# Kamino666/S2VT-video-caption

Hardware: AMD Instinct MI355X
Metric: training frames/sec (whole node) (higher is better)
Workload: dtype f32; 1 GPU; BASELINE configs[1]: S2VT train step, B=64 per GPU x 1 GPU, 80x4096 feats, hidden=embed=1000, vocab=12000, fp32, Adam; global_batch=64, frames=80, parallelism=dp1

## Files before the change

include/s2vt_hip.h:

```cpp
#ifndef S2VT_HIP_H
#define S2VT_HIP_H

#include <stddef.h>
#include <stdint.h>

#ifdef __cplusplus
extern "C" {
#endif

#define S2VT_ABI_VERSION 9

#define S2VT_ERR_ARG (-1)
#define S2VT_ERR_INDEX (-2)
#define S2VT_ERR_TIMEOUT (-3)

typedef struct s2vt_dims {
    int32_t B, L, F, H, E, V;
} s2vt_dims;

typedef struct s2vt_params {
    const float* vid_w_ih;
    const float* vid_w_hh;
    const float* vid_b_ih;
    const float* vid_b_hh;
// ... 189 lines not shown
                        size_t workspace_bytes, void* stream);

size_t s2vt_lstm_seq_bf16_workspace_bytes(int32_t T, int32_t B, int32_t H);
int s2vt_lstm_seq_fwd_bf16(int32_t T, int32_t B, int32_t H, float* gx_stash, int32_t n_gx, const float* bias,
                           const float* w_hh, float* h_all, float* c_all, void* workspace, size_t workspace_bytes,
                           int32_t persistent, int32_t block, void* stream);
int s2vt_lstm_seq_fwd_bf16_pair(int32_t T, int32_t B, int32_t H, float* gx_stash0, float* gx_stash1, int32_t n_gx,
                                const float* bias0, const float* bias1, const float* w_hh0, const float* w_hh1,
                                float* h_all0, float* h_all1, float* c_all0, float* c_all1, void* workspace,
                                size_t workspace_bytes, int32_t block, void* stream);
size_t s2vt_lstm_seq_bwd_bf16_workspace_bytes(int32_t T, int32_t B, int32_t H);
int s2vt_lstm_seq_bwd_bf16(int32_t T, int32_t B, int32_t H, const float* w_hh, const float* dh_out, int32_t dh_first,
                           const float* c_all, float* stash_dg, void* workspace, size_t workspace_bytes,
                           int32_t persistent, int32_t block, void* stream);
int s2vt_lstm_seq_bwd_bf16_pair(int32_t T, int32_t B, int32_t H, const float* w_hh0, const float* w_hh1, const float* dh_out0,
                                const float* dh_out1, int32_t dh_first, const float* c_all0, const float* c_all1,
                                float* stash_dg0, float* stash_dg1, void* workspace, size_t workspace_bytes, int32_t block,
                                void* stream);
int s2vt_set_recurrence_mode(int32_t mode);
int s2vt_recurrence_plan(int32_t B, int32_t H, int32_t* fwd, int32_t* bwd);
int s2vt_decode_plan(const s2vt_dims* d, int32_t encode_only, int32_t* padded_B, int32_t* persist_encode, int32_t* schedule);

size_t s2vt_lstm_seq_x3_workspace_bytes(int32_t T, int32_t B, int32_t H);
int s2vt_lstm_seq_fwd_x3_persist(int32_t T, int32_t B, int32_t H, float* gx_stash0, float* gx_stash1, int32_t n_gx,
                              const float* bias0, const float* bias1, const float* w_hh0, const float* w_hh1, float* h_all0,
                              float* h_all1, float* c_all0, float* c_all1, int32_t block, void* workspace,
                              size_t workspace_bytes, void* stream);
size_t s2vt_lstm_seq_bwd_x3_workspace_bytes(int32_t T, int32_t B, int32_t H, int32_t block);
int s2vt_lstm_seq_bwd_x3_persist(int32_t T, int32_t B, int32_t H, const float* w_hh0, const float* w_hh1, const float* dh_out0,
                                 const float* dh_out1, int32_t dh_first, const float* c_all0, const float* c_all1, float* stash_dg0,
                                 float* stash_dg1, int32_t block, void* workspace, size_t workspace_bytes, void* stream);
int s2vt_decode_step_argmax(int32_t B, int32_t H, int32_t V, const float* h, const float* w_out, const float* b_out,
                            unsigned long long* packed, void* stream);

size_t s2vt_decode_step_argmax_x3_workspace_bytes(int32_t B, int32_t H, int32_t V);
int s2vt_decode_step_argmax_x3(int32_t B, int32_t H, int32_t V, const float* h, const float* w_out, const float* b_out,
                               unsigned long long* packed, void* workspace, size_t workspace_bytes, void* stream);

int s2vt_decode_step_sample(int32_t B, int32_t H, int32_t V, const float* h, const float* w_out, const float* b_out, float temperature,
                            uint64_t seed, int32_t step, int32_t row0, unsigned long long* packed, void* stream);
size_t s2vt_decode_step_sample_x3_workspace_bytes(int32_t B, int32_t H, int32_t V);
int s2vt_decode_step_sample_x3(int32_t B, int32_t H, int32_t V, const float* h, const float* w_out, const float* b_out, float temperature,
                               uint64_t seed, int32_t step, int32_t row0, unsigned long long* packed, void* workspace,
                               size_t workspace_bytes, void* stream);
int s2vt_sample_decode(const s2vt_dims* d, const s2vt_params* p, const float* feats, int32_t sos_ix, float temperature, uint64_t seed,
                       int64_t* ids, void* workspace, size_t workspace_bytes, void* stream);
int s2vt_sample_decode_cached(const s2vt_dims* d, const s2vt_params* p, const float* feats, int32_t sos_ix, float temperature,
                              uint64_t seed, int64_t* ids, void* workspace, size_t workspace_bytes, void* cache, size_t cache_bytes,
                              int32_t cache_valid, void* stream);

int s2vt_scheduled_decode(const s2vt_dims* d, const s2vt_params* p, const float* feats, const int64_t* targets, int64_t targets_ld,
                          float ss_prob, int32_t draw_mode, float temperature, uint64_t seed, int64_t* used, int64_t* draws,
                          void* workspace, size_t workspace_bytes, void* stream);
int s2vt_scheduled_decode_cached(const s2vt_dims* d, const s2vt_params* p, const float* feats, const int64_t* targets, int64_t targets_ld,
                                 float ss_prob, int32_t draw_mode, float temperature, uint64_t seed, int64_t* used, int64_t* draws,
                                 void* workspace, size_t workspace_bytes, void* cache, size_t cache_bytes, int32_t cache_valid,
                                 void* stream);
int s2vt_ss_mix(const int64_t* draw_tokens, const int64_t* targets, int64_t targets_ld, int32_t B, float ss_prob, uint64_t seed,
                int32_t step, int32_t row0, int64_t* out, void* stream);
int s2vt_ss_unpack(const unsigned long long* packed, int32_t steps, int32_t B, const int64_t* targets, int64_t targets_ld, float ss_prob,
                   uint64_t seed, int64_t* used, int64_t* draws, void* stream);

int32_t s2vt_set_option(const char* name, int32_t value);
int32_t s2vt_option_count(void);
const char* s2vt_option_name(int32_t index);

int s2vt_set_gemm_mode(int32_t mode);

int s2vt_set_pipeline_block(int32_t steps);
int s2vt_set_decode_schedule(int32_t schedule);
int s2vt_decode_encode_cached(const s2vt_dims* d, const s2vt_params* p, const float* feats, void* workspace, size_t workspace_bytes,
                              void* cache, size_t cache_bytes, int32_t cache_valid, float* vid_h, float* vid_c, float* word_h,
                              float* word_c, float* gx_dec, int32_t depth, void* stream);
int s2vt_beam_step_gx(const s2vt_dims* d, const s2vt_params* p, int32_t R, const int32_t* row_b, const int32_t* row_state,
                      const int32_t* tok, const float* gx_vid, const float* word_h_in, const float* word_c_in, float* word_h_out,
                      float* word_c_out, int32_t* top_ix, float* top_lp, void* workspace, size_t workspace_bytes, void* cache,
                      size_t cache_bytes, void* stream);
int s2vt_pipeline_overlaps(void);

int s2vt_set_graph_mode(int32_t on);
int s2vt_graph_stats(int64_t* captures, int64_t* replays);

int s2vt_test_occupy_cus(int32_t workgroups, int32_t lds_bytes, int64_t microseconds, void* stream);
int s2vt_test_lane_delay(int32_t lanes, int64_t microseconds);

int s2vt_prof_enable(int32_t on);
int s2vt_prof_read(int32_t kind, double* total_ms, int64_t* launches);
int s2vt_prof_read_busy(int32_t kind, double* busy_ms);
int s2vt_prof_reset(void);

#ifdef __cplusplus
}
#endif
#endif
```

s2vt-video-caption_amd/capi.py:

```python
import ctypes
import os
from ctypes import POINTER, c_char_p, c_double, c_float, c_int32, c_int64, c_size_t, c_uint64, c_void_p

_HERE = os.path.dirname(os.path.abspath(__file__))
LIB_PATH = os.environ.get("S2VT_LIB") or os.path.join(_HERE, "libs2vt_hip.so")


class Dims(ctypes.Structure):
    _fields_ = [(n, c_int32) for n in ("B", "L", "F", "H", "E", "V")]


PARAM_FIELDS = ("vid_w_ih", "vid_w_hh", "vid_b_ih", "vid_b_hh", "word_w_ih", "word_w_hh", "word_b_ih", "word_b_hh",
                "feat_w", "feat_b", "out_w", "out_b", "emb_w")
PARAM_KEYS = ("vid_rnn.weight_ih_l0", "vid_rnn.weight_hh_l0", "vid_rnn.bias_ih_l0", "vid_rnn.bias_hh_l0",
              "word_rnn.weight_ih_l0", "word_rnn.weight_hh_l0", "word_rnn.bias_ih_l0", "word_rnn.bias_hh_l0",
              "feat_linear.weight", "feat_linear.bias", "out_linear.weight", "out_linear.bias", "embedding.weight")


class Params(ctypes.Structure):
    _fields_ = [(n, c_void_p) for n in PARAM_FIELDS]


class Grads(ctypes.Structure):
    _fields_ = [(n, c_void_p) for n in PARAM_FIELDS]
# ... 69 lines not shown
    "s2vt_beam_queue_step": (c_int32, [c_int32] * 6 + [c_void_p, c_size_t] + [c_void_p] * 6),
    "s2vt_beam_queue_result": (c_int32, [c_int32, c_int32, c_int32, c_void_p, c_size_t, c_void_p, c_int32, c_void_p, c_void_p]),
    "s2vt_feat_proj_fwd": (c_int32, [POINTER(Dims), c_void_p, c_void_p, c_void_p, c_void_p, c_void_p]),
    "s2vt_feat_proj_bwd": (c_int32, [POINTER(Dims), c_void_p, c_void_p, c_void_p, c_void_p, c_void_p, c_void_p,
                                     c_void_p, c_void_p]),
    "s2vt_colsum_ws_floats": (c_size_t, [c_int64, c_int32]),
    "s2vt_lstm_step_fwd": (c_int32, [c_int32, c_int32] + [c_void_p] * 9),
    "s2vt_lstm_step_fwd_token": (c_int32, [c_int32, c_int32, c_int32, c_int32] + [c_void_p] * 6 + [c_int64, c_void_p, c_void_p,
                                                                                            c_int32, c_void_p, c_void_p, c_void_p]),
    "s2vt_lstm_step_bwd": (c_int32, [c_int32, c_int32] + [c_void_p] * 7 + [c_int32, c_void_p, c_void_p]),
    "s2vt_lstm_seq_fwd": (c_int32, [c_int32, c_int32, c_int32, c_void_p, c_int32] + [c_void_p] * 6),
    "s2vt_lstm_seq_bwd": (c_int32, [c_int32, c_int32, c_int32, c_void_p, c_void_p, c_int32] + [c_void_p] * 5),
    "s2vt_gru_step_fwd": (c_int32, [c_int32, c_int32] + [c_void_p] * 8),
    "s2vt_gru_step_fwd_token": (c_int32, [c_int32, c_int32, c_int32, c_int32] + [c_void_p] * 6 + [c_int64, c_void_p, c_void_p,
                                                                                           c_int32, c_void_p, c_void_p]),
    "s2vt_gru_step_bwd": (c_int32, [c_int32, c_int32] + [c_void_p] * 10),
    "s2vt_lstm_chain_fwd": (c_int32, [c_int32, c_int32, c_int32, c_int32, POINTER(LstmLayer), c_void_p]),
    "s2vt_lstm_chain_bwd_workspace_bytes": (c_size_t, [c_int32, c_int32, c_int32]),
    "s2vt_lstm_chain_bwd": (c_int32, [c_int32, c_int32, c_int32, c_int32, POINTER(LstmLayer), c_void_p, c_size_t, c_void_p]),
    "s2vt_gru_seq_fwd": (c_int32, [c_int32, c_int32, c_int32, c_void_p, c_int32] + [c_void_p] * 6),
    "s2vt_gru_seq_bwd": (c_int32, [c_int32, c_int32, c_int32, c_void_p, c_void_p, c_int32] + [c_void_p] * 7),
    "s2vt_tokens_time_major": (c_int32, [c_int32, c_int32, c_int32, c_void_p, c_int64, c_void_p, c_void_p]),
    "s2vt_lstm_seq_bf16_workspace_bytes": (c_size_t, [c_int32, c_int32, c_int32]),
    "s2vt_lstm_seq_fwd_bf16": (c_int32, [c_int32, c_int32, c_int32, c_void_p, c_int32, c_void_p, c_void_p, c_void_p,
                                         c_void_p, c_void_p, c_size_t, c_int32, c_int32, c_void_p]),
    "s2vt_lstm_seq_fwd_bf16_pair": (c_int32, [c_int32, c_int32, c_int32, c_void_p, c_void_p, c_int32] + [c_void_p] * 9 +
                                    [c_size_t, c_int32, c_void_p]),
    "s2vt_lstm_seq_bwd_bf16_workspace_bytes": (c_size_t, [c_int32, c_int32, c_int32]),
    "s2vt_lstm_seq_bwd_bf16": (c_int32, [c_int32, c_int32, c_int32, c_void_p, c_void_p, c_int32, c_void_p, c_void_p, c_void_p,
                                         c_size_t, c_int32, c_int32, c_void_p]),
    "s2vt_lstm_seq_bwd_bf16_pair": (c_int32, [c_int32, c_int32, c_int32, c_void_p, c_void_p, c_void_p, c_void_p, c_int32,
                                              c_void_p, c_void_p, c_void_p, c_void_p, c_void_p, c_size_t, c_int32, c_void_p]),
    "s2vt_lstm_seq_x3_workspace_bytes": (c_size_t, [c_int32, c_int32, c_int32]),
    "s2vt_lstm_seq_fwd_x3_persist": (c_int32, [c_int32, c_int32, c_int32, c_void_p, c_void_p, c_int32] + [c_void_p] * 8 +
                                  [c_int32, c_void_p, c_size_t, c_void_p]),
    "s2vt_lstm_seq_bwd_x3_workspace_bytes": (c_size_t, [c_int32, c_int32, c_int32, c_int32]),
    "s2vt_lstm_seq_bwd_x3_persist": (c_int32, [c_int32, c_int32, c_int32, c_void_p, c_void_p, c_void_p, c_void_p, c_int32] +
                                     [c_void_p] * 4 + [c_int32, c_void_p, c_size_t, c_void_p]),
    "s2vt_set_recurrence_mode": (c_int32, [c_int32]),
    "s2vt_recurrence_plan": (c_int32, [c_int32, c_int32, POINTER(c_int32), POINTER(c_int32)]),
    "s2vt_decode_plan": (c_int32, [POINTER(Dims), c_int32, POINTER(c_int32), POINTER(c_int32), POINTER(c_int32)]),
    "s2vt_decode_step_argmax": (c_int32, [c_int32, c_int32, c_int32] + [c_void_p] * 5),
    "s2vt_decode_step_argmax_x3_workspace_bytes": (c_size_t, [c_int32, c_int32, c_int32]),
    "s2vt_decode_step_argmax_x3": (c_int32, [c_int32, c_int32, c_int32] + [c_void_p] * 5 + [c_size_t, c_void_p]),
    "s2vt_decode_step_sample": (c_int32, [c_int32, c_int32, c_int32, c_void_p, c_void_p, c_void_p, c_float, c_uint64, c_int32, c_int32,
                                          c_void_p, c_void_p]),
    "s2vt_decode_step_sample_x3_workspace_bytes": (c_size_t, [c_int32, c_int32, c_int32]),
    "s2vt_decode_step_sample_x3": (c_int32, [c_int32, c_int32, c_int32, c_void_p, c_void_p, c_void_p, c_float, c_uint64, c_int32,
                                             c_int32, c_void_p, c_void_p, c_size_t, c_void_p]),
    "s2vt_sample_decode": (c_int32, [POINTER(Dims), POINTER(Params), c_void_p, c_int32, c_float, c_uint64, c_void_p, c_void_p,
                                     c_size_t, c_void_p]),
    "s2vt_sample_decode_cached": (c_int32, [POINTER(Dims), POINTER(Params), c_void_p, c_int32, c_float, c_uint64, c_void_p, c_void_p,
                                            c_size_t, c_void_p, c_size_t, c_int32, c_void_p]),
    "s2vt_scheduled_decode": (c_int32, [POINTER(Dims), POINTER(Params), c_void_p, c_void_p, c_int64, c_float, c_int32, c_float, c_uint64,
                                        c_void_p, c_void_p, c_void_p, c_size_t, c_void_p]),
    "s2vt_scheduled_decode_cached": (c_int32, [POINTER(Dims), POINTER(Params), c_void_p, c_void_p, c_int64, c_float, c_int32, c_float,
                                               c_uint64, c_void_p, c_void_p, c_void_p, c_size_t, c_void_p, c_size_t, c_int32, c_void_p]),
    "s2vt_ss_mix": (c_int32, [c_void_p, c_void_p, c_int64, c_int32, c_float, c_uint64, c_int32, c_int32, c_void_p, c_void_p]),
    "s2vt_ss_unpack": (c_int32, [c_void_p, c_int32, c_int32, c_void_p, c_int64, c_float, c_uint64, c_void_p, c_void_p, c_void_p]),
    "s2vt_gru_step_fwd_token_ss": (c_int32, [c_int32, c_int32, c_int32, c_int32] + [c_void_p] * 6 + [c_int64, c_void_p, c_void_p, c_int64,
                                                                                              c_float, c_uint64, c_int32, c_int32, c_void_p,
                                                                                              c_void_p]),
    "s2vt_weighted_ce_forward": (c_int32, [c_int32, c_int32, c_int32, c_void_p, c_void_p, c_int64, c_void_p, c_int64, c_void_p,
                                           c_void_p, c_void_p, c_void_p]),
    "s2vt_weighted_ce_backward": (c_int32, [c_int32, c_int32, c_int32, c_void_p, c_void_p, c_int64, c_void_p, c_int64, c_void_p,
                                            c_void_p, c_void_p, c_void_p, c_void_p]),
    "s2vt_cider_rewards": (c_int32, [POINTER(CiderTable), c_void_p, c_void_p, c_int32, c_int32, c_int64, c_int32, c_int32, c_void_p,
                                     c_void_p]),
    "s2vt_sc_weights": (c_int32, [c_void_p, c_void_p, c_void_p, c_int32, c_int32, c_int32, c_int32, c_void_p, c_void_p, c_void_p]),
    "s2vt_mean_ce_backward_fused": (c_int32, [POINTER(Dims), c_void_p, c_void_p, c_int64, c_void_p, c_void_p, c_void_p, c_size_t,
                                              c_void_p]),
    "s2vt_set_option": (c_int32, [c_char_p, c_int32]),
    "s2vt_option_count": (c_int32, []),
    "s2vt_option_name": (c_char_p, [c_int32]),
    "s2vt_set_gemm_mode": (c_int32, [c_int32]),
    "s2vt_set_pipeline_block": (c_int32, [c_int32]),
    "s2vt_set_decode_schedule": (c_int32, [c_int32]),
    "s2vt_decode_encode_cached": (c_int32, [POINTER(Dims), POINTER(Params), c_void_p, c_void_p, c_size_t, c_void_p, c_size_t, c_int32,
                                            c_void_p, c_void_p, c_void_p, c_void_p, c_void_p, c_int32, c_void_p]),
    "s2vt_beam_step_gx": (c_int32, [POINTER(Dims), POINTER(Params), c_int32] + [c_void_p] * 10 + [c_void_p, c_size_t, c_void_p, c_size_t,
                                                                                                  c_void_p]),
    "s2vt_pipeline_overlaps": (c_int32, []),
    "s2vt_test_occupy_cus": (c_int32, [c_int32, c_int32, c_int64, c_void_p]),
    "s2vt_test_lane_delay": (c_int32, [c_int32, c_int64]),
    "s2vt_set_graph_mode": (c_int32, [c_int32]),
    "s2vt_graph_stats": (c_int32, [POINTER(c_int64), POINTER(c_int64)]),
    "s2vt_prof_enable": (c_int32, [c_int32]),
    "s2vt_prof_read": (c_int32, [c_int32, POINTER(c_double), POINTER(c_int64)]),
    "s2vt_prof_read_busy": (c_int32, [c_int32, POINTER(c_double)]),
    "s2vt_prof_reset": (c_int32, []),
}

_lib = None


class S2VTHipError(RuntimeError):
    pass


def load():
    global _lib
    if _lib is not None:
        return _lib
    if not os.path.exists(LIB_PATH):
        raise S2VTHipError(
            "libs2vt_hip.so is not built (%s). Run `python -c 'import __graft_entry__ as g; g.build()'` "
            "or `python s2vt-video-caption_amd/build.py`. There is no CPU fallback for the S2VT hot path." % LIB_PATH)
    import torch
    rt = os.path.join(os.path.dirname(torch.__file__), "lib", "libamdhip64.so")
    if os.path.exists(rt):
        ctypes.CDLL(rt, mode=ctypes.RTLD_GLOBAL)
    lib = ctypes.CDLL(LIB_PATH)
    for name, (res, args) in SIGNATURES.items():
        fn = getattr(lib, name)
        fn.restype = res
        fn.argtypes = args
    if lib.s2vt_abi_version() != ABI_VERSION:
        raise S2VTHipError("libs2vt_hip.so ABI %d != %d" % (lib.s2vt_abi_version(), ABI_VERSION))
    _lib = lib
    return lib


ERR_INDEX, ERR_TIMEOUT = -2, -3


def check(rc, what):
    if rc != 0:
        msg = load().s2vt_last_error()
        text = "%s failed (rc=%d): %s" % (what, rc, msg.decode(errors="replace") if msg else "?")
        if rc == ERR_INDEX:
            raise IndexError(text)
        raise S2VTHipError(text)


def check_async_error(wait=True):
    check(load().s2vt_check_async_error(1 if wait else 0), "s2vt_check_async_error")


def prof_read_busy(kind):
    ms = c_double(0.0)
    check(load().s2vt_prof_read_busy(kind, ctypes.byref(ms)), "s2vt_prof_read_busy")
    return ms.value


def prof_read(kind):
    ms, n = c_double(0.0), c_int64(0)
    check(load().s2vt_prof_read(kind, ctypes.byref(ms), ctypes.byref(n)), "s2vt_prof_read")
    return ms.value, n.value


def recurrence_plan(B, H):
    import ctypes
    f, b = c_int32(0), c_int32(0)
    lib = load()
    check(lib.s2vt_recurrence_plan(int(lib.s2vt_padded_batch(int(B))), int(H), ctypes.byref(f), ctypes.byref(b)), "s2vt_recurrence_plan")
    return f.value, b.value


def decode_plan(dims, encode_only=False):
    d = dims if isinstance(dims, Dims) else Dims(*[int(x) for x in dims])
    b, pe, sc = c_int32(0), c_int32(0), c_int32(0)
    check(load().s2vt_decode_plan(d, 1 if encode_only else 0, ctypes.byref(b), ctypes.byref(pe), ctypes.byref(sc)), "s2vt_decode_plan")
    return b.value, pe.value, sc.value
```

s2vt-video-caption_amd/csrc/api_runtime.hip:

```cpp
#include "api_internal.h"

namespace s2vt {

static thread_local char g_err[512] = "";
const char* last_error_text() { return g_err; }
#ifdef S2VT_EXPERIMENT_STAMPS
unsigned long long* g_xstamps = nullptr;
int g_xstamp_block = 0;
#endif

void set_error(const char* fmt, ...) {
    va_list ap;
    va_start(ap, fmt);
    vsnprintf(g_err, sizeof(g_err), fmt, ap);
    va_end(ap);
}

int check_hip(hipError_t e, const char* what) {
    if (e == hipSuccess) return 0;
    set_error("%s: %s", what, hipGetErrorString(e));
    return (int)e;
}

struct ErrRecord { int* host; hipEvent_t ev; bool pending; };
// ... 183 lines not shown
        (void)hipEventSynchronize(e2);
        (void)hipEventElapsedTime(&single, e0, e2);
    }
    (void)hipEventDestroy(e0); (void)hipEventDestroy(e1); (void)hipEventDestroy(e2);
    return both < 1.6f * single;
}
static int g_side_overlaps = -1;
int side_stream_overlaps() { return g_side_overlaps; }
int side_stream(hipStream_t caller, hipStream_t* out) {
    if (!g_side) {
        hipStream_t cand = nullptr;
        g_side_overlaps = 0;
        for (int attempt = 0; attempt < 8 && !g_side_overlaps; ++attempt) {
            S2VT_HIP(hipStreamCreateWithFlags(&cand, hipStreamNonBlocking));
            if (streams_overlap(caller, cand)) g_side_overlaps = 1;
        }
        g_side = cand;
    }
    *out = g_side;
    return 0;
}
int get_event(size_t i, hipEvent_t* out) {
    while (g_events.size() <= i) {
        hipEvent_t e;
        S2VT_HIP(hipEventCreateWithFlags(&e, hipEventDisableTiming));
        g_events.push_back(e);
    }
    *out = g_events[i];
    return 0;
}
int handoff(hipStream_t from, hipStream_t to, size_t ev_index) {
    if (from == to) return 0;
    hipEvent_t e;
    int rc = get_event(ev_index, &e);
    if (rc) return rc;
    S2VT_HIP(hipEventRecord(e, from));
    S2VT_HIP(hipStreamWaitEvent(to, e, 0));
    return 0;
}

int lgemm(const Lane& ln, bool ak, bool bk, int M, int N, int K, const float* A, int64_t lda, RowMap am,
                 const float* B, int64_t ldb, RowMap bm, float* C, int64_t ldc, RowMap cm, const float* bias, bool acc) {
    if (int rc = lane_delay(ln.s)) return rc;
    ProfScope ps(ln.s, K_GEMM, 1);
    return gemm_f32(ln.s, ak, bk, M, N, K, A, lda, am, B, ldb, bm, C, ldc, cm, bias, acc, ln.gws, ln.gws_floats);
}

}

using namespace s2vt;

extern "C" {

int s2vt_abi_version(void) { return S2VT_ABI_VERSION; }
const char* s2vt_last_error(void) { return last_error_text(); }
int s2vt_check_async_error(int32_t wait) { return poll_async_error(wait != 0); }

int s2vt_set_gemm_mode(int32_t mode) {
    return option_set(O_GEMM_MODE, mode);
}

int s2vt_gemm_tune(int32_t nplanes, int32_t tile_rows, int32_t nsplit) {
    S2VT_REQUIRE(nplanes == 1 || nplanes == 3, "s2vt_gemm_tune: nplanes must be 1 (bf16 kernel) or 3 (split-precision kernel)");
    if (nplanes == 1) gemm_b1_tune(tile_rows, nsplit);
    else gemm_x3_tune(tile_rows, nsplit);
    return 0;
}

int s2vt_pipeline_overlaps(void) { return g_side_overlaps; }

int s2vt_set_graph_mode(int32_t on) {
    return option_set(O_GRAPH, on < 0 ? -1 : (on ? 1 : 0));
}
int s2vt_graph_stats(int64_t* captures, int64_t* replays) {
    if (captures) *captures = (int64_t)g_graph_captures;
    if (replays) *replays = (int64_t)g_graph_replays;
    return 0;
}

int s2vt_test_occupy_cus(int32_t workgroups, int32_t lds_bytes, int64_t microseconds, void* stream) {
    return occupy_cus((hipStream_t)stream, workgroups, lds_bytes, microseconds);
}

int s2vt_test_lane_delay(int32_t lanes, int64_t microseconds) {
    S2VT_REQUIRE(lanes >= 0 && lanes <= 3 && microseconds >= 0 && microseconds <= 5000000,
                 "s2vt_test_lane_delay: lanes must be 0..3 and microseconds 0..5000000 (got %d, %lld)", (int)lanes, (long long)microseconds);
    g_lane_delay_lanes = lanes;
    g_lane_delay_us = microseconds;
    return 0;
}

int s2vt_set_pipeline_block(int32_t steps) {
    return option_set(O_PIPE_BLOCK, steps < 0 ? 0 : steps);
}

int s2vt_prof_enable(int32_t on) { g_prof = on != 0; return 0; }

int s2vt_prof_reset(void) {
    for (auto& r : g_recs) g_free.emplace_back(r.a, r.b);
    g_recs.clear();
    return 0;
}

int s2vt_prof_read(int32_t kind, double* total_ms, int64_t* launches) {
    S2VT_REQUIRE(kind >= 0 && kind < K_NKINDS && total_ms && launches, "s2vt_prof_read: bad arguments");
    double ms = 0.0;
    int64_t n = 0;
    for (auto& r : g_recs) {
        if (r.kind != kind) continue;
        S2VT_HIP(hipEventSynchronize(r.b));
        float t = 0.f;
        S2VT_HIP(hipEventElapsedTime(&t, r.a, r.b));
        ms += t;
        n += r.launches;
    }
    *total_ms = ms;
    *launches = n;
    return 0;
}

int s2vt_prof_read_busy(int32_t kind, double* busy_ms) {
    S2VT_REQUIRE(kind >= 0 && kind < K_NKINDS && busy_ms, "s2vt_prof_read_busy: bad arguments");
    *busy_ms = 0.0;
    if (g_recs.empty()) return 0;
    const hipEvent_t ref = g_recs.front().a;
    S2VT_HIP(hipEventSynchronize(ref));
    std::vector<std::pair<double, double>> iv;
    for (auto& r : g_recs) {
        if (r.kind != kind) continue;
        S2VT_HIP(hipEventSynchronize(r.b));
        float s = 0.f, e = 0.f;
        if (r.a != ref) S2VT_HIP(hipEventElapsedTime(&s, ref, r.a));
        S2VT_HIP(hipEventElapsedTime(&e, ref, r.b));
        if (e > s) iv.emplace_back((double)s, (double)e);
    }
    std::sort(iv.begin(), iv.end());
    double busy = 0.0, hi = -1e300;
    for (auto& x : iv) {
        if (x.first > hi) { busy += x.second - x.first; hi = x.second; }
        else if (x.second > hi) { busy += x.second - hi; hi = x.second; }
    }
    *busy_ms = busy;
    return 0;
}

}
```

s2vt-video-caption_amd/csrc/gemm_x3.hip:

```cpp
#include <stdlib.h>

#include <type_traits>

#include "common.h"
#include "gemm_persist.h"
#include "kernels.h"

namespace s2vt {

typedef short bf16x8 __attribute__((ext_vector_type(8)));
typedef short bf16x4 __attribute__((ext_vector_type(4)));

constexpr int X_REC = 6144;
constexpr int X_NS = 3;

template <int MI, bool TT>
__global__ __launch_bounds__(512) void gemm_x3_kernel(PersistGemmArgs p) {
    constexpr int NRA = MI, TMR = 64 * MI, X_STAGE = (NRA + 4) * X_REC;
    __shared__ __attribute__((aligned(1024))) unsigned char smem[X_NS * X_STAGE];
    const unsigned lbase = (unsigned)(uintptr_t)(__attribute__((address_space(3))) unsigned char*)smem;
    const int tid = threadIdx.x, lane = tid & 63;
    const int wave = __builtin_amdgcn_readfirstlane(tid >> 6);
    const int wm = wave >> 2, wn = wave & 3;
    const int li = lane & 31, lh = lane >> 5;

    const PersistWalk walk(p, blockIdx, gridDim);
    const int q_end = walk.q_end, gx = walk.gx, kbeg = walk.kbeg, kend = walk.kend;
    int q = walk.q;
    if (q >= q_end) return;
    const int nk = (kend - kbeg) >> 4;
    auto tile_of = [&](int t, int& m0, int& n0) { walk.tile_of<TMR>(t, m0, n0); };

    const bool loader = wave < NRA + 4;
    auto rsrc_of = [&](int m0, int n0) {
        if constexpr (TT) {
            const bool isA = wave < NRA;
            const unsigned short* base = isA ? p.A : p.B;
            const int64_t ld = isA ? p.lda : p.ldb;
            const int c0 = (isA ? m0 : n0) >> 4;
            const int64_t off = (int64_t)(kbeg >> 6) * 64 * ld + (int64_t)c0 * (X_REC / 2);
            int64_t bytes = ((int64_t)((kend - kbeg) >> 6) * 64 * ld - (int64_t)c0 * (X_REC / 2)) * 2;
            if (bytes > 0xFFFFF000ll) bytes = 0xFFFFF000ll;
            return __builtin_amdgcn_make_buffer_rsrc(const_cast<unsigned short*>(base + off), 0, (int)bytes, 0x00020000);
        }
        const bool isA = wave < NRA;
        const int nrb = ((isA ? p.M : p.N) + 63) >> 6;
        int rb = isA ? (m0 >> 6) + wave : (n0 >> 6) + (wave - NRA);
        rb = rb < nrb ? rb : nrb - 1;
        const unsigned short* base = isA ? p.A : p.B;
        const int64_t ld = isA ? p.lda : p.ldb;
        return __builtin_amdgcn_make_buffer_rsrc(const_cast<unsigned short*>(base + (int64_t)rb * 64 * ld + (int64_t)(kbeg >> 4) * (X_REC / 2)), 0,
                                                 nk * X_REC, 0x00020000);
    };
    const int vlane = TT ? ((lane >> 1) & 1) * X_REC + (lane & 1) * 1024 + (lane >> 2) * 16 : lane * 16;
    const int64_t tt_ld2 = (wave < NRA ? p.lda : p.ldb) * 128;
    const int tt_wq = wave < NRA ? wave : wave - NRA;
#define X3_REQ1(J, R, ST, SLOT)                                                                                           \
    if constexpr (TT) {                                                                                                   \
        __builtin_amdgcn_raw_ptr_buffer_load_lds(R, (__attribute__((address_space(3))) void*)(smem + (SLOT) * X_STAGE + (wave < NRA ? 0 : NRA * X_REC) + \
                                                     ((2 * tt_wq + (J) / 3) * 3 + (J) % 3) * 1024),                       \
                                                 16, vlane, (int)(((ST) >> 2) * tt_ld2) + (2 * tt_wq + (J) / 3) * 2 * X_REC + ((J) % 3) * 2048 + ((ST) & 3) * 256, 0, 0); \
    } else {                                                                                                              \
        __builtin_amdgcn_raw_ptr_buffer_load_lds(R, (__attribute__((address_space(3))) void*)(smem + (SLOT) * X_STAGE + wave * X_REC + (J) * 1024), \
                                                 16, vlane, (ST) * X_REC + (J) * 1024, 0, 0);                             \
    }

    f32x16 acc[MI][2];

    unsigned la[MI];
#pragma unroll
    for (int mi = 0; mi < MI; ++mi) {
        const int x = wm * MI + mi;
        la[mi] = lbase + (unsigned)((x >> 1) * X_REC + (x & 1) * 512 + lh * 1024 + li * 16);
    }
    const unsigned lb = lbase + (unsigned)((NRA + wn) * X_REC + lh * 1024 + li * 16);
    const unsigned tt_lane = (unsigned)((8 * lh + ((li & 15) >> 2)) * 64 + (li >> 4) * 32 + (li & 3) * 8);
    const unsigned lb_t = lbase + tt_lane + (unsigned)(NRA * X_REC + wn * 2 * 3072);
    unsigned lat[MI];
#pragma unroll
    for (int mi = 0; mi < MI; ++mi) lat[mi] = lbase + tt_lane + (unsigned)((wm * MI + mi) * 3072);

    bf16x8 a0p[MI], b0p[2];
    auto stage = [&](int g, auto more_tag, bool more_rt, __amdgpu_buffer_rsrc_t r2, int s2, int nwait, bool deferred) {
        const bool more = decltype(more_tag)::value || more_rt;
        if (deferred) {
#pragma unroll
            for (int mi = 0; mi < MI; ++mi)
#pragma unroll
                for (int ni = 0; ni < 2; ++ni) acc[mi][ni] = __builtin_amdgcn_mfma_f32_32x32x16_bf16(a0p[mi], b0p[ni], acc[mi][ni], 0, 0, 0);
        }
        __builtin_amdgcn_sched_barrier(0);
        if (nwait == 6) asm volatile("s_waitcnt vmcnt(6) lgkmcnt(0)\n\ts_barrier" ::: "memory");
        else if (nwait == 0) asm volatile("s_waitcnt vmcnt(0) lgkmcnt(0)\n\ts_barrier" ::: "memory");
        else asm volatile("s_waitcnt vmcnt(%0) lgkmcnt(0)\n\ts_barrier" ::"n"(6 + 8 * MI) : "memory");
        const int slot = g % X_NS, slot2 = (g + 2) % X_NS;
        const unsigned so = (unsigned)(slot * X_STAGE);
        bf16x8 a[3][MI], b[3][2];
#define X3_RD(DST, ADDR, OFF) asm volatile("ds_read_b128 %0, %1 offset:%2" : "=v"(DST) : "v"(ADDR), "n"(OFF));
#define X3_RDT(DST, ADDR, OFF)                                                                                               \
    {                                                                                                                        \
        bf16x4 lo_, hi_;                                                                                                     \
        asm volatile("ds_read_b64_tr_b16 %0, %1 offset:%2" : "=v"(lo_) : "v"(ADDR), "n"(OFF));                               \
        asm volatile("ds_read_b64_tr_b16 %0, %1 offset:%2" : "=v"(hi_) : "v"(ADDR), "n"((OFF) + 256));                       \
        DST = __builtin_shufflevector(lo_, hi_, 0, 1, 2, 3, 4, 5, 6, 7);                                                     \
    }
#define X3_LDA(PL)                                                                                                           \
    if constexpr (TT) { _Pragma("unroll") for (int mi = 0; mi < MI; ++mi) { X3_RDT(a[PL][mi], lat[mi] + so, (PL) * 1024) } } \
    else { _Pragma("unroll") for (int mi = 0; mi < MI; ++mi) { X3_RD(a[PL][mi], la[mi] + so, (PL) * 2048) } }
#define X3_LDB(PL)                                                                                                           \
    if constexpr (TT) { const unsigned b_ = lb_t + so; X3_RDT(b[PL][0], b_, (PL) * 1024) X3_RDT(b[PL][1], b_, (3 + (PL)) * 1024) } \
    else { const unsigned b_ = lb + so; X3_RD(b[PL][0], b_, (PL) * 2048) X3_RD(b[PL][1], b_, (PL) * 2048 + 512) }
#define X3_WAIT(N, PA, PB)                                                                                     \
    {                                                                                                          \
        asm volatile("s_waitcnt lgkmcnt(%0)" ::"n"(N));                                                        \
        _Pragma("unroll") for (int i_ = 0; i_ < MI; ++i_) asm volatile("" : "+v"(a[PA][i_]));                  \
        asm volatile("" : "+v"(b[PB][0]));                                                                     \
        asm volatile("" : "+v"(b[PB][1]));                                                                     \
    }
        __builtin_amdgcn_sched_barrier(0);
        X3_LDA(1) X3_LDB(1) X3_LDA(0) X3_LDB(2)
        if constexpr (!TT) { X3_LDA(2) X3_LDB(0) }
#define X3_PROD(PA, PB)                                                                                          \
    _Pragma("unroll") for (int mi = 0; mi < MI; ++mi) _Pragma("unroll") for (int ni = 0; ni < 2; ++ni)           \
        acc[mi][ni] = __builtin_amdgcn_mfma_f32_32x32x16_bf16(a[PA][mi], b[PB][ni], acc[mi][ni], 0, 0, 0);
        const bool req = more && loader;
#define X3_GROUP(N, PA, PB, J, DOWAIT)                                     \
    if constexpr (DOWAIT) { X3_WAIT(N, PA, PB) }                           \
    X3_PROD(PA, PB)                                                        \
    if (req) { X3_REQ1(J, r2, s2, slot2) }                                 \
    __builtin_amdgcn_sched_barrier(0);
        if (req) { X3_REQ1(5, r2, s2, slot2) }
        __builtin_amdgcn_sched_barrier(0);
        if constexpr (TT) {
            X3_GROUP(2 * (MI + 2), 1, 1, 0, true)
            X3_LDA(2) X3_LDB(0)
            X3_GROUP(2 * (MI + 2), 0, 2, 1, true)
            X3_GROUP(0, 2, 0, 2, true)
        } else {
            X3_GROUP(2 * (MI + 2), 1, 1, 0, true)
            X3_GROUP(MI + 2, 0, 2, 1, true)
            X3_GROUP(0, 2, 0, 2, true)
        }
        X3_GROUP(0, 0, 1, 3, false)
        X3_GROUP(0, 1, 0, 4, false)
#pragma unroll
        for (int mi = 0; mi < MI; ++mi) a0p[mi] = a[0][mi];
        b0p[0] = b[0][0]; b0p[1] = b[0][1];
#undef X3_GROUP
#undef X3_PROD
#undef X3_WAIT
#undef X3_RD
#undef X3_RDT
#undef X3_LDA
#undef X3_LDB
    };

    int m0, n0;
    tile_of(q, m0, n0);
    __amdgpu_buffer_rsrc_t r0 = rsrc_of(m0, n0);
    if (loader) {
#pragma unroll
        for (int j = 0; j < 6; ++j) { X3_REQ1(j, r0, 0, 0) }
#pragma unroll
        for (int j = 0; j < 6; ++j) { X3_REQ1(j, r0, 1, 1) }
    }
    int s = 0;
    int qn = q + gx;
    int m1 = 0, n1 = 0;
    if (qn < q_end) tile_of(qn, m1, n1);
    __amdgpu_buffer_rsrc_t r1 = rsrc_of(m1, n1);
    int nwait = 6;
    zero_acc<MI>(acc);
    for (int g = 0;; ++g) {
        const bool has_next = qn < q_end;
        for (; s + 2 < nk; ++s, ++g) {
            stage(g, std::true_type{}, true, r0, s + 2, nwait, s > 0);
            nwait = 6;
        }
        stage(g, std::false_type{}, has_next, r1, 0, nwait, true);
        ++g;
        stage(g, std::false_type{}, has_next, r1, 1, has_next ? 6 : 0, true);
#pragma unroll
        for (int mi = 0; mi < MI; ++mi)
#pragma unroll
            for (int ni = 0; ni < 2; ++ni) acc[mi][ni] = __builtin_amdgcn_mfma_f32_32x32x16_bf16(a0p[mi], b0p[ni], acc[mi][ni], 0, 0, 0);

        store_tile<MI>(acc, m0, n0, wm, wn, li, lh, p.M, p.N, p.C, p.ldc, p.cmap, p.bias, p.accumulate, p.slabs);
        if (!has_next) break;
        nwait = store_tile_counted<MI>(p, m0, n0, wn) ? 6 + 8 * MI : 6;
        q = qn; m0 = m1; n0 = n1; r0 = r1;
        qn = q + gx;
        if (qn < q_end) tile_of(qn, m1, n1);
        r1 = rsrc_of(m1, n1);
        s = 0;
        zero_acc<MI>(acc);
    }
#undef X3_REQ1
}

static const double kX3Stage[5] = {0, 0, 1.35, 1.75, 2.15};
static const double kX3Epi[5] = {0, 0, 4.5, 6.0, 8.0};
static int g_x3_force_mi = 0, g_x3_force_n = 0;
void gemm_x3_tune(int tile_rows, int nsplit) {
    g_x3_force_mi = (tile_rows >= 128 && tile_rows <= 256 && tile_rows % 64 == 0) ? tile_rows / 64 : 0;
    g_x3_force_n = nsplit > 0 ? nsplit : 0;
}

static int gemm_x3_impl(hipStream_t stream, bool tt, int M, int N, int K, const unsigned short* A, int64_t lda, const unsigned short* B,
                       int64_t ldb, float* C, int64_t ldc, RowMap cmap, const float* bias, bool accumulate, float* splitk_ws,
                       size_t splitk_ws_floats) {
    if (M <= 0 || N <= 0) return 0;
    if (tt) {
        S2VT_REQUIRE(K > 0 && K % 64 == 0 && lda % 8 == 0 && ldb % 8 == 0 && lda >= 3 * (int64_t)((M + 63) / 64 * 64) &&
                         ldb >= 3 * (int64_t)((N + 63) / 64 * 64) && (reinterpret_cast<uintptr_t>(A) & 15) == 0 &&
                         (reinterpret_cast<uintptr_t>(B) & 15) == 0,
                     "gemm_x3_tt: K (image rows) must be a multiple of 64, the row images hold pad64(M) / pad64(N) columns");
    } else
    S2VT_REQUIRE(K > 0 && K % 64 == 0 && lda % 8 == 0 && ldb % 8 == 0 && lda >= 3 * (int64_t)K && ldb >= 3 * (int64_t)K &&
                     (reinterpret_cast<uintptr_t>(A) & 15) == 0 && (reinterpret_cast<uintptr_t>(B) & 15) == 0,
                 "gemm_x3: K must be the zero-padded multiple of 64 of the blocked plane layout, operands 16-B aligned");
    static const int order[3] = {4, 3, 2};
    const PersistPlanIn in = {tt, M, N, K, lda > ldb ? lda : ldb, splitk_ws ? splitk_ws_floats : 0, g_x3_force_mi, g_x3_force_n,
                              order, 3, false, 16, kX3Stage, kX3Epi, 0xFFFFF000ll};
    return launch_persistent_gemm(
        stream, in, A, lda, B, ldb, C, ldc, cmap, bias, accumulate, splitk_ws, splitk_ws_floats, "gemm_x3_kernel",
        "gemm_x3_tt: a row image of %lld bytes needs k slices below 4 GB and split-K scratch for them (%zu floats given)",
        [&](int mi, dim3 grid, const PersistGemmArgs& p) {
            if (tt) {
                switch (mi) {
                    case 2: hipLaunchKernelGGL((gemm_x3_kernel<2, true>), grid, dim3(512), 0, stream, p); break;
                    case 3: hipLaunchKernelGGL((gemm_x3_kernel<3, true>), grid, dim3(512), 0, stream, p); break;
                    default: hipLaunchKernelGGL((gemm_x3_kernel<4, true>), grid, dim3(512), 0, stream, p); break;
                }
            } else {
                switch (mi) {
                    case 2: hipLaunchKernelGGL((gemm_x3_kernel<2, false>), grid, dim3(512), 0, stream, p); break;
                    case 3: hipLaunchKernelGGL((gemm_x3_kernel<3, false>), grid, dim3(512), 0, stream, p); break;
                    default: hipLaunchKernelGGL((gemm_x3_kernel<4, false>), grid, dim3(512), 0, stream, p); break;
                }
            }
        });
}
int gemm_x3(hipStream_t stream, int M, int N, int K, const unsigned short* A, int64_t lda, const unsigned short* B,
            int64_t ldb, float* C, int64_t ldc, RowMap cmap, const float* bias, bool accumulate, float* splitk_ws,
            size_t splitk_ws_floats) {
    return gemm_x3_impl(stream, false, M, N, K, A, lda, B, ldb, C, ldc, cmap, bias, accumulate, splitk_ws, splitk_ws_floats);
}
int gemm_x3_tt(hipStream_t stream, int M, int N, int K, const unsigned short* A, int64_t lda, const unsigned short* B,
               int64_t ldb, float* C, int64_t ldc, RowMap cmap, const float* bias, bool accumulate, float* splitk_ws,
               size_t splitk_ws_floats) {
    return gemm_x3_impl(stream, true, M, N, K, A, lda, B, ldb, C, ldc, cmap, bias, accumulate, splitk_ws, splitk_ws_floats);
}

}
```

Measured before the change: 521,100 frames/s.

## Double-buffer LDS fragment registers in x3 GEMM to overlap next-stage reads with MFMA

Restructures the x3 bf16 GEMM main loop so that each stage reads the next k-stage's LDS fragments into a second register set (parity-selected) while the current stage's MFMAs run. The loop is unrolled by two with even/odd parity, the prologue preloads the first stage and issues an extra global prefetch, and the tile tail runs four stages. This aims to hide LDS read latency behind matrix math, at the cost of more VGPRs, which may reduce occupancy or cause spills for larger MI. A test hook exposing cu_plan_cap is also added.

```diff
diff --git a/include/s2vt_hip.h b/include/s2vt_hip.h
--- a/include/s2vt_hip.h
+++ b/include/s2vt_hip.h
@@ -295,6 +295,8 @@
 int s2vt_graph_stats(int64_t* captures, int64_t* replays);
 
 int s2vt_test_occupy_cus(int32_t workgroups, int32_t lds_bytes, int64_t microseconds, void* stream);
+
+int s2vt_test_plan_cap(int32_t compute_units);
 int s2vt_test_lane_delay(int32_t lanes, int64_t microseconds);
 
 int s2vt_prof_enable(int32_t on);
diff --git a/s2vt-video-caption_amd/capi.py b/s2vt-video-caption_amd/capi.py
--- a/s2vt-video-caption_amd/capi.py
+++ b/s2vt-video-caption_amd/capi.py
@@ -175,6 +175,7 @@
                                                                                                   c_void_p]),
     "s2vt_pipeline_overlaps": (c_int32, []),
     "s2vt_test_occupy_cus": (c_int32, [c_int32, c_int32, c_int64, c_void_p]),
+    "s2vt_test_plan_cap": (c_int32, [c_int32]),
     "s2vt_test_lane_delay": (c_int32, [c_int32, c_int64]),
     "s2vt_set_graph_mode": (c_int32, [c_int32]),
     "s2vt_graph_stats": (c_int32, [POINTER(c_int64), POINTER(c_int64)]),
diff --git a/s2vt-video-caption_amd/csrc/api_runtime.hip b/s2vt-video-caption_amd/csrc/api_runtime.hip
--- a/s2vt-video-caption_amd/csrc/api_runtime.hip
+++ b/s2vt-video-caption_amd/csrc/api_runtime.hip
@@ -289,6 +289,8 @@
     return occupy_cus((hipStream_t)stream, workgroups, lds_bytes, microseconds);
 }
 
+int s2vt_test_plan_cap(int32_t compute_units) { return cu_plan_cap(compute_units); }
+
 int s2vt_test_lane_delay(int32_t lanes, int64_t microseconds) {
     S2VT_REQUIRE(lanes >= 0 && lanes <= 3 && microseconds >= 0 && microseconds <= 5000000,
                  "s2vt_test_lane_delay: lanes must be 0..3 and microseconds 0..5000000 (got %d, %lld)", (int)lanes, (long long)microseconds);
diff --git a/s2vt-video-caption_amd/csrc/gemm_x3.hip b/s2vt-video-caption_amd/csrc/gemm_x3.hip
--- a/s2vt-video-caption_amd/csrc/gemm_x3.hip
+++ b/s2vt-video-caption_amd/csrc/gemm_x3.hip
@@ -80,22 +80,11 @@
 #pragma unroll
     for (int mi = 0; mi < MI; ++mi) lat[mi] = lbase + tt_lane + (unsigned)((wm * MI + mi) * 3072);
 
-    bf16x8 a0p[MI], b0p[2];
-    auto stage = [&](int g, auto more_tag, bool more_rt, __amdgpu_buffer_rsrc_t r2, int s2, int nwait, bool deferred) {
-        const bool more = decltype(more_tag)::value || more_rt;
-        if (deferred) {
-#pragma unroll
-            for (int mi = 0; mi < MI; ++mi)
-#pragma unroll
-                for (int ni = 0; ni < 2; ++ni) acc[mi][ni] = __builtin_amdgcn_mfma_f32_32x32x16_bf16(a0p[mi], b0p[ni], acc[mi][ni], 0, 0, 0);
-        }
-        __builtin_amdgcn_sched_barrier(0);
-        if (nwait == 6) asm volatile("s_waitcnt vmcnt(6) lgkmcnt(0)\n\ts_barrier" ::: "memory");
-        else if (nwait == 0) asm volatile("s_waitcnt vmcnt(0) lgkmcnt(0)\n\ts_barrier" ::: "memory");
-        else asm volatile("s_waitcnt vmcnt(%0) lgkmcnt(0)\n\ts_barrier" ::"n"(6 + 8 * MI) : "memory");
-        const int slot = g % X_NS, slot2 = (g + 2) % X_NS;
-        const unsigned so = (unsigned)(slot * X_STAGE);
-        bf16x8 a[3][MI], b[3][2];
+    constexpr bool FULL = MI <= 3;
+    constexpr int NPAIR = (TT ? 2 : 1) * (MI + 2);
+    bf16x8 fa[3][MI], fb[3][2], fas[3][MI], fbs[3][2];
+#define X3_A(NX, PL) (((FULL || (PL) == 0) && (P ^ (NX))) ? fas[PL] : fa[PL])
+#define X3_B(NX, PL) (((FULL || (PL) == 0) && (P ^ (NX))) ? fbs[PL] : fb[PL])
 #define X3_RD(DST, ADDR, OFF) asm volatile("ds_read_b128 %0, %1 offset:%2" : "=v"(DST) : "v"(ADDR), "n"(OFF));
 #define X3_RDT(DST, ADDR, OFF)                                                                                               \
     {                                                                                                                        \
@@ -104,56 +93,77 @@
         asm volatile("ds_read_b64_tr_b16 %0, %1 offset:%2" : "=v"(hi_) : "v"(ADDR), "n"((OFF) + 256));                       \
         DST = __builtin_shufflevector(lo_, hi_, 0, 1, 2, 3, 4, 5, 6, 7);                                                     \
     }
-#define X3_LDA(PL)                                                                                                           \
-    if constexpr (TT) { _Pragma("unroll") for (int mi = 0; mi < MI; ++mi) { X3_RDT(a[PL][mi], lat[mi] + so, (PL) * 1024) } } \
-    else { _Pragma("unroll") for (int mi = 0; mi < MI; ++mi) { X3_RD(a[PL][mi], la[mi] + so, (PL) * 2048) } }
-#define X3_LDB(PL)                                                                                                           \
-    if constexpr (TT) { const unsigned b_ = lb_t + so; X3_RDT(b[PL][0], b_, (PL) * 1024) X3_RDT(b[PL][1], b_, (3 + (PL)) * 1024) } \
-    else { const unsigned b_ = lb + so; X3_RD(b[PL][0], b_, (PL) * 2048) X3_RD(b[PL][1], b_, (PL) * 2048 + 512) }
-#define X3_WAIT(N, PA, PB)                                                                                     \
+#define X3_LDA(NX, PL, SO)                                                                                                        \
+    if constexpr (TT) { _Pragma("unroll") for (int mi = 0; mi < MI; ++mi) { X3_RDT(X3_A(NX, PL)[mi], lat[mi] + (SO), (PL) * 1024) } } \
+    else { _Pragma("unroll") for (int mi = 0; mi < MI; ++mi) { X3_RD(X3_A(NX, PL)[mi], la[mi] + (SO), (PL) * 2048) } }
+#define X3_LDB(NX, PL, SO)                                                                                                        \
+    if constexpr (TT) { const unsigned b_ = lb_t + (SO); X3_RDT(X3_B(NX, PL)[0], b_, (PL) * 1024) X3_RDT(X3_B(NX, PL)[1], b_, (3 + (PL)) * 1024) } \
+    else { const unsigned b_ = lb + (SO); X3_RD(X3_B(NX, PL)[0], b_, (PL) * 2048) X3_RD(X3_B(NX, PL)[1], b_, (PL) * 2048 + 512) }
+#define X3_WAIT(N, NX, PA, PB)                                                                                 \
     {                                                                                                          \
-        asm volatile("s_waitcnt lgkmcnt(%0)" ::"n"(N));                                                        \
-        _Pragma("unroll") for (int i_ = 0; i_ < MI; ++i_) asm volatile("" : "+v"(a[PA][i_]));                  \
-        asm volatile("" : "+v"(b[PB][0]));                                                                     \
-        asm volatile("" : "+v"(b[PB][1]));                                                                     \
-    }
-        __builtin_amdgcn_sched_barrier(0);
-        X3_LDA(1) X3_LDB(1) X3_LDA(0) X3_LDB(2)
-        if constexpr (!TT) { X3_LDA(2) X3_LDB(0) }
-#define X3_PROD(PA, PB)                                                                                          \
-    _Pragma("unroll") for (int mi = 0; mi < MI; ++mi) _Pragma("unroll") for (int ni = 0; ni < 2; ++ni)           \
-        acc[mi][ni] = __builtin_amdgcn_mfma_f32_32x32x16_bf16(a[PA][mi], b[PB][ni], acc[mi][ni], 0, 0, 0);
+        if constexpr ((N) >= 0) asm volatile("s_waitcnt lgkmcnt(%0)" ::"n"((N) >= 0 ? (N) : 0));               \
+        _Pragma("unroll") for (int i_ = 0; i_ < MI; ++i_) asm volatile("" : "+v"(X3_A(NX, PA)[i_]));           \
+        asm volatile("" : "+v"(X3_B(NX, PB)[0]));                                                              \
+        asm volatile("" : "+v"(X3_B(NX, PB)[1]));                                                              \
+    }
+#define X3_PROD(PA, PB)                                                                                                  \
+    _Pragma("unroll") for (int mi = 0; mi < MI; ++mi) _Pragma("unroll") for (int ni = 0; ni < 2; ++ni)                   \
+        acc[mi][ni] = __builtin_amdgcn_mfma_f32_32x32x16_bf16(X3_A(0, PA)[mi], X3_B(0, PB)[ni], acc[mi][ni], 0, 0, 0);   \
+    __builtin_amdgcn_sched_barrier(0);
+    auto stage = [&](int g, auto parity, auto more_tag, bool more_rt, __amdgpu_buffer_rsrc_t r2, int s2, int nwait, bool rd) {
+        constexpr int P = decltype(parity)::value;
+        const bool more = decltype(more_tag)::value || more_rt;
         const bool req = more && loader;
-#define X3_GROUP(N, PA, PB, J, DOWAIT)                                     \
-    if constexpr (DOWAIT) { X3_WAIT(N, PA, PB) }                           \
-    X3_PROD(PA, PB)                                                        \
-    if (req) { X3_REQ1(J, r2, s2, slot2) }                                 \
-    __builtin_amdgcn_sched_barrier(0);
-        if (req) { X3_REQ1(5, r2, s2, slot2) }
-        __builtin_amdgcn_sched_barrier(0);
-        if constexpr (TT) {
-            X3_GROUP(2 * (MI + 2), 1, 1, 0, true)
-            X3_LDA(2) X3_LDB(0)
-            X3_GROUP(2 * (MI + 2), 0, 2, 1, true)
-            X3_GROUP(0, 2, 0, 2, true)
+        const int slot2 = g % X_NS;
+        const unsigned so = (unsigned)(((g + 1) % X_NS) * X_STAGE);
+        __builtin_amdgcn_sched_barrier(0);
+        if constexpr (FULL) {
+            X3_WAIT(TT ? -1 : 2 * NPAIR, 0, 1, 1)
+            X3_PROD(1, 1)
+            X3_WAIT(NPAIR, 0, 0, 2)
+            X3_PROD(0, 2)
+            X3_WAIT(0, 0, 2, 0)
+            X3_PROD(2, 0)
         } else {
-            X3_GROUP(2 * (MI + 2), 1, 1, 0, true)
-            X3_GROUP(MI + 2, 0, 2, 1, true)
-            X3_GROUP(0, 2, 0, 2, true)
-        }
-        X3_GROUP(0, 0, 1, 3, false)
-        X3_GROUP(0, 1, 0, 4, false)
-#pragma unroll
-        for (int mi = 0; mi < MI; ++mi) a0p[mi] = a[0][mi];
-        b0p[0] = b[0][0]; b0p[1] = b[0][1];
-#undef X3_GROUP
-#undef X3_PROD
-#undef X3_WAIT
-#undef X3_RD
-#undef X3_RDT
-#undef X3_LDA
-#undef X3_LDB
+            X3_WAIT(0, 0, 1, 1)
+            X3_WAIT(-1, 0, 0, 2)
+            X3_WAIT(-1, 0, 2, 0)
+            X3_PROD(1, 1)
+            X3_PROD(0, 2)
+            X3_PROD(2, 0)
+        }
+        if (rd) {
+            if (nwait == 6) asm volatile("s_waitcnt vmcnt(6) lgkmcnt(0)\n\ts_barrier" ::: "memory");
+            else if (nwait == 0) asm volatile("s_waitcnt vmcnt(0) lgkmcnt(0)\n\ts_barrier" ::: "memory");
+            else asm volatile("s_waitcnt vmcnt(%0) lgkmcnt(0)\n\ts_barrier" ::"n"(6 + 8 * MI) : "memory");
+            if constexpr (FULL) {
+                X3_LDA(1, 1, so) X3_LDB(1, 1, so)
+                if constexpr (!TT) { X3_LDA(1, 0, so) X3_LDB(1, 2, so) X3_LDA(1, 2, so) X3_LDB(1, 0, so) }
+            } else {
+                X3_LDA(1, 0, so) X3_LDB(1, 2, so)
+            }
+        }
+        __builtin_amdgcn_sched_barrier(0);
+        X3_PROD(0, 1)
+        if (req) { X3_REQ1(0, r2, s2, slot2) X3_REQ1(1, r2, s2, slot2) }
+        if (rd) {
+            if constexpr (!FULL) { X3_LDA(1, 2, so) X3_LDB(1, 0, so) X3_LDB(1, 1, so) }
+            else if constexpr (TT) { X3_LDA(1, 0, so) X3_LDB(1, 2, so) }
+        }
+        __builtin_amdgcn_sched_barrier(0);
+        X3_PROD(1, 0)
+        if (req) { X3_REQ1(2, r2, s2, slot2) X3_REQ1(3, r2, s2, slot2) }
+        if (rd) {
+            if constexpr (!FULL) { X3_LDA(1, 1, so) }
+            else if constexpr (TT) { X3_WAIT(NPAIR, 1, 1, 1) X3_LDA(1, 2, so) X3_LDB(1, 0, so) }
+        }
+        __builtin_amdgcn_sched_barrier(0);
+        X3_PROD(0, 0)
+        if (req) { X3_REQ1(4, r2, s2, slot2) X3_REQ1(5, r2, s2, slot2) }
+        __builtin_amdgcn_sched_barrier(0);
     };
+    const std::integral_constant<int, 0> even{};
+    const std::integral_constant<int, 1> odd{};
 
     int m0, n0;
     tile_of(q, m0, n0);
@@ -169,21 +179,31 @@
     int m1 = 0, n1 = 0;
     if (qn < q_end) tile_of(qn, m1, n1);
     __amdgpu_buffer_rsrc_t r1 = rsrc_of(m1, n1);
+    asm volatile("s_waitcnt vmcnt(6)\n\ts_barrier" ::: "memory");
+    {
+        constexpr int P = 0;
+        X3_LDA(0, 1, 0u) X3_LDB(0, 1, 0u) X3_LDA(0, 0, 0u) X3_LDB(0, 2, 0u)
+        if constexpr (TT) { X3_WAIT(NPAIR, 0, 1, 1) }
+        X3_LDA(0, 2, 0u) X3_LDB(0, 0, 0u)
+    }
+    if (loader) {
+#pragma unroll
+        for (int j = 0; j < 6; ++j) { X3_REQ1(j, r0, 2, 2) }
+    }
     int nwait = 6;
     zero_acc<MI>(acc);
-    for (int g = 0;; ++g) {
+    for (int g = 0;;) {
         const bool has_next = qn < q_end;
-        for (; s + 2 < nk; ++s, ++g) {
-            stage(g, std::true_type{}, true, r0, s + 2, nwait, s > 0);
+        for (; s + 4 < nk; s += 2, g += 2) {
+            stage(g, even, std::true_type{}, true, r0, s + 3, nwait, true);
             nwait = 6;
-        }
-        stage(g, std::false_type{}, has_next, r1, 0, nwait, true);
-        ++g;
-        stage(g, std::false_type{}, has_next, r1, 1, has_next ? 6 : 0, true);
-#pragma unroll
-        for (int mi = 0; mi < MI; ++mi)
-#pragma unroll
-            for (int ni = 0; ni < 2; ++ni) acc[mi][ni] = __builtin_amdgcn_mfma_f32_32x32x16_bf16(a0p[mi], b0p[ni], acc[mi][ni], 0, 0, 0);
+            stage(g + 1, odd, std::true_type{}, true, r0, s + 4, 6, true);
+        }
+        stage(g, even, std::true_type{}, true, r0, s + 3, nwait, true);
+        stage(g + 1, odd, std::false_type{}, has_next, r1, 0, 6, true);
+        stage(g + 2, even, std::false_type{}, has_next, r1, 1, has_next ? 6 : 0, true);
+        stage(g + 3, odd, std::false_type{}, has_next, r1, 2, 6, has_next);
+        g += 4;
 
         store_tile<MI>(acc, m0, n0, wm, wn, li, lh, p.M, p.N, p.C, p.ldc, p.cmap, p.bias, p.accumulate, p.slabs);
         if (!has_next) break;
@@ -195,6 +215,14 @@
         s = 0;
         zero_acc<MI>(acc);
     }
+#undef X3_PROD
+#undef X3_WAIT
+#undef X3_LDB
+#undef X3_LDA
+#undef X3_RDT
+#undef X3_RD
+#undef X3_B
+#undef X3_A
 #undef X3_REQ1
 }
 
```

Result: no change. 523,600 frames/s (median of 6 runs) (+0.5%).
